# gersteinlab/REPIC-copy

Hardware: AMD Instinct MI355X
Metric: micrographs/sec (get_cliques, whole node) at 1/2/4/8 MI355X; % HBM roofline (higher is better)
Workload: dtype f64; 1 GPU; C2: {'k': 3, 'n_true': 300, 'box': 180, 'width': 4096, 'height': 4096, 'keep': 0.9, 'jit': 0.08, 'fp': 0.1}; micrographs_per_gpu=10000, scaling=weak, k=3, box_size=180, boxes_per_gpu=9030947, edges_per_gpu=11401310, cliques_per_gpu=5244495, parallelism=dp1 (micrograph shards), io=HBM-resident, steps_in_flight=3, streams=3

## Files before the change

repic-copy_amd/csrc/rgc_device.h:

```cpp
#pragma once
#pragma clang fp contract(off)
#include <hip/hip_runtime.h>
#include <stdint.h>
#include <math.h>

#include "pyset.h"

namespace rgc {

constexpr int WG = 256;
constexpr int NW = WG / 64;

template <typename T>
using gptr = __attribute__((address_space(1))) T*;
#if defined(RGC_STAMPS)
template <typename T>
__device__ __forceinline__ gptr<T> gdetach(T* p) { return (gptr<T>)p; }
__device__ __forceinline__ double sdetach(double v) { return v; }
__device__ __forceinline__ int sdetach(int v) { return v; }
__device__ __forceinline__ int64_t sdetach(int64_t v) { return v; }
#else
template <typename T>
__device__ __forceinline__ gptr<T> gdetach(T* p) {
  uint64_t v = (uint64_t)p, r;
// ... 124 lines not shown
  float r;
  asm("v_min_f32 %0, %1, %2" : "=v"(r) : "v"(a), "v"(b));
  return r;
}
__device__ __forceinline__ float wave_incl_min_f32(float v) {
  const int inf = 0x7f800000;
#define RGC_DPP_MIN(ctrl, rm, bc)                                                          \
  v = vmin_f32(v, __int_as_float(__builtin_amdgcn_update_dpp(inf, __float_as_int(v), ctrl, \
                                                             rm, 0xf, bc)))
  RGC_DPP_MIN(0x111, 0xf, false);
  RGC_DPP_MIN(0x112, 0xf, false);
  RGC_DPP_MIN(0x114, 0xf, false);
  RGC_DPP_MIN(0x118, 0xf, false);
  RGC_DPP_MIN(0x142, 0xa, false);
  RGC_DPP_MIN(0x143, 0xc, false);
#undef RGC_DPP_MIN
  return v;
}

template <int BS, typename A>
__device__ __forceinline__ int block_scan_dpp32(A* a, int n, int* lds) {
  constexpr bool PAIRS = sizeof(A) == 2;
  const int per0 = (n + BS - 1) / BS;
  const int per = PAIRS ? (per0 + 1) & ~1 : per0;
  const int c0 = min((int)threadIdx.x * per, n), c1 = min(c0 + per, n);
  uint32_t* a2 = reinterpret_cast<uint32_t*>(a);
  const int ce = PAIRS ? c0 + ((c1 - c0) & ~1) : c1;
  int s = 0;
  if constexpr (PAIRS) {
    for (int c = c0; c < ce; c += 2) {
      const uint32_t v = a2[c >> 1];
      s += (int)(v & 0xFFFFu) + (int)(v >> 16);
    }
    if (ce < c1) s += a[ce];
  } else {
    for (int c = c0; c < c1; ++c) s += a[c];
  }
  const int l = threadIdx.x & 63, w = threadIdx.x >> 6;
  const int inc = wave_incl_add32(s);
  if (l == 63) lds[w] = inc;
  __syncthreads();
  int pre = inc - s, tot = 0;
#pragma unroll
  for (int i = 0; i < BS / 64; ++i) {
    const int x = lds[i];
    pre += (i < w) ? x : 0;
    tot += x;
  }
  if constexpr (PAIRS) {
    for (int c = c0; c < ce; c += 2) {
      const uint32_t v = a2[c >> 1];
      const int p1 = pre + (int)(v & 0xFFFFu);
      a2[c >> 1] = ((uint32_t)pre & 0xFFFFu) | ((uint32_t)p1 << 16);
      pre = p1 + (int)(v >> 16);
    }
    if (ce < c1) a[ce] = (A)pre;
  } else {
    for (int c = c0; c < c1; ++c) {
      const int v = a[c];
      a[c] = (A)pre;
      pre += v;
    }
  }
  if (threadIdx.x == BS - 1) a[n] = (A)tot;
  __syncthreads();
  return tot;
}

template <int BS, typename T>
__device__ __forceinline__ T block_excl_scan_dpp(T v, T* lds, T* total) {
  const int l = threadIdx.x & 63, w = threadIdx.x >> 6;
  const T inc = wave_incl_scan(v, [](T a, T b) { return a + b; });
  if (l == 63) lds[w] = inc;
  __syncthreads();
  T pre = 0, tot = 0;
#pragma unroll
  for (int i = 0; i < BS / 64; ++i) {
    const T x = lds[i];
    pre += (i < w) ? x : (T)0;
    tot += x;
  }
  *total = tot;
  return pre + inc - v;
}

template <int BS, typename A>
__device__ __forceinline__ int64_t block_scan_dpp(A* a, int n, int64_t* lds) {
  const int per = (n + BS - 1) / BS;
  const int c0 = min((int)threadIdx.x * per, n), c1 = min(c0 + per, n);
  int64_t s = 0;
  for (int c = c0; c < c1; ++c) s += a[c];
  int64_t tot;
  int64_t pre = block_excl_scan_dpp<BS>(s, lds, &tot);
  for (int c = c0; c < c1; ++c) {
    const A v = a[c];
    a[c] = (A)pre;
    pre += v;
  }
  if (threadIdx.x == BS - 1) a[n] = (A)tot;
  __syncthreads();
  return tot;
}

template <int BS = WG>
__device__ __forceinline__ int64_t block_excl_scan(int64_t v, int64_t* lds, int64_t* total) {
  const int l = threadIdx.x & 63, w = threadIdx.x >> 6;
  int64_t inc = v;
  for (int o = 1; o < 64; o <<= 1) {
    const int64_t t = __shfl_up(inc, o, 64);
    if (l >= o) inc += t;
  }
  __syncthreads();
  if (l == 63) lds[w] = inc;
  __syncthreads();
  int64_t pre = 0, tot = 0;
  for (int i = 0; i < BS / 64; ++i) {
    if (i < w) pre += lds[i];
    tot += lds[i];
  }
  *total = tot;
  return pre + inc - v;
}

template <int BS = WG>
__device__ __forceinline__ int64_t block_scan_array(uint32_t* a, int n, int64_t* lds) {
  const int per = (n + BS - 1) / BS;
  const int c0 = min((int)threadIdx.x * per, n), c1 = min(c0 + per, n);
  int64_t s = 0;
  for (int c = c0; c < c1; ++c) s += a[c];
  int64_t tot;
  int64_t pre = block_excl_scan<BS>(s, lds, &tot);
  for (int c = c0; c < c1; ++c) {
    const uint32_t v = a[c];
    a[c] = (uint32_t)pre;
    pre += v;
  }
  __syncthreads();
  return tot;
}

template <int BS = WG>
__device__ __forceinline__ int64_t block_scan_u16(uint16_t* a, int n, int64_t* lds) {
  const int per = (n + BS - 1) / BS;
  const int c0 = min((int)threadIdx.x * per, n), c1 = min(c0 + per, n);
  int64_t s = 0;
  for (int c = c0; c < c1; ++c) s += a[c];
  int64_t tot;
  int64_t pre = block_excl_scan<BS>(s, lds, &tot);
  for (int c = c0; c < c1; ++c) {
    const uint16_t v = a[c];
    a[c] = (uint16_t)pre;
    pre += v;
  }
  __syncthreads();
  return tot;
}

__host__ __device__ __forceinline__ double overlap(double x, double y, double a, double b, double B) {
  const double xo = fmax((fmin(x, a) + B) - fmax(x, a), 0.0);
  const double yo = fmax((fmin(y, b) + B) - fmax(y, b), 0.0);
  return xo * yo;
}

__host__ __device__ __forceinline__ double jaccard(double x, double y, double a, double b, double B,
                                          double two_b2) {
  const double xo = fmax((fmin(x, a) + B) - fmax(x, a), 0.0);
// ... 241 lines not shown
```

repic-copy_amd/csrc/rgc_fused.hip:

```cpp
#pragma clang fp contract(off)

#include <type_traits>

#ifdef RGC_STAMPS
#include <hip/hip_runtime.h>
namespace rgc {
__shared__ unsigned long long g_bwait[16];
__device__ __forceinline__ void raw_barrier() {
  __builtin_amdgcn_fence(__ATOMIC_RELEASE, "workgroup");
  __builtin_amdgcn_s_barrier();
  __builtin_amdgcn_fence(__ATOMIC_ACQUIRE, "workgroup");
}
__device__ __forceinline__ void timed_barrier() {
  const unsigned long long t0 = __builtin_amdgcn_s_memtime();
  raw_barrier();
  if ((threadIdx.x & 63) == 0) g_bwait[threadIdx.x >> 6] += __builtin_amdgcn_s_memtime() - t0;
}
}
#define __syncthreads() ::rgc::timed_barrier()
#endif

#include "rgc_device.h"
#include "rgc_kernels.h"

namespace rgc {

constexpr int MAXW = 16;
constexpr int fused_rb(int nt) { return nt <= 256 ? 4 : nt >= 1024 ? 5 : 2; }
enum : unsigned { TWO_P1 = 1, TWO_P2C = 2, TWO_P3A = 4, TWO_P3B = 8, TWO_P5 = 16, TWO_P6A = 32 };
#ifndef RGC_TWO_MASK
#define RGC_TWO_MASK 0u
#endif
constexpr unsigned fused_two(int k, bool wide, int nt) {
  unsigned m = RGC_TWO_MASK;
  if (fused_rb(nt) != 2) m &= ~TWO_P1;
  if (k >= 4) m &= ~TWO_P5;
  return m;
}

struct FusedHdr {
  union {
    struct {
      double redd[MAXW];
      int64_t red64[MAXW];
      uint64_t redu[MAXW];
      int redi[MAXW];
    };
    double red4[4][MAXW];
  };
  double minx, miny, cell, inv_cell, inv_celly;
  double xbs;
  float inv_gy;
  int gx, gy, ncell, nkey;
  int E, nodes, cc_cnt, cc_max, target, V, status;
  uint32_t ccur;
  int tief[2];
  int qslot;
  int64_t C, base;
};

__host__ __device__ inline int fused_cells(int nmax) { return nmax <= 2048 ? 4 * nmax : 2 * nmax; }

__host__ __device__ inline int fwd_blocks(int nmax) { return (nmax + 63) / 64; }

__host__ __device__ inline FusedLayout fused_layout(int nmax, int ecap, bool wide) {
  FusedLayout L;
  auto al = [](int v) { return (v + 15) & ~15; };
  int o = al((int)sizeof(FusedHdr));
  L.off_sxy = o; o += al((wide ? 16 : 8) * nmax);
  L.off_cnt = o; o += al(4 * (nmax + 4));
  L.off_fwd = o; o += al(2 * (fwd_blocks(nmax) * 65 + 4));
  L.off_pos = o; o += al(2 * nmax);
  L.off_vrank = o; o += al(2 * nmax);
  L.off_dst = o; o += al(2 * ecap);
  L.off_union = o;
  L.off_cstart = o; o += al(2 * (fused_cells(nmax) + 8));
  L.off_parent = o; o += al(2 * (nmax + 8));
  L.off_scell = o; o += al(2 * nmax);
  L.off_citems = o; o += al(2 * nmax);
  L.off_flags = o; o += al(nmax);
  L.off_smark = o;
  L.total = o;
  L.off_cbuf = L.off_cstart;
  return L;
}

int fused_lds_bytes(int nmax, int ecap, bool wide) { return fused_layout(nmax, ecap, wide).total; }

struct FShared {
  void* sxy;
  uint16_t* cstart;
  uint32_t* cnt;
  uint16_t* fwd;
  uint16_t* bend;
  uint16_t* parent;
  uint16_t* citems;
  uint16_t* pos;
  uint16_t* scell;
  uint16_t* vrank;
  uint8_t* flags;
  uint16_t* dst;
  uint16_t* split;
  uint16_t* cbuf;
  double* vscore;
  bool vstaged;
  __device__ __forceinline__ int eb(int i) const { return fwd[i]; }
  __device__ __forceinline__ int ee(int i) const {
    return (i & 63) == 63 ? bend[i >> 6] : fwd[i + 1];
  }
};

template <bool W>
__device__ __forceinline__ double2 ld_xy(const FShared& S, int t) {
  if constexpr (W) {
    return reinterpret_cast<const double2*>(S.sxy)[t];
  } else {
    const float2 f = reinterpret_cast<const float2*>(S.sxy)[t];
    return make_double2((double)f.x, (double)f.y);
  }
}
template <bool W>
// ... 416 lines not shown
        for (int i = 0; i < K; ++i) e[4 + i] = c.b0 + li[i];
      }
      if (tie) return;
    } else {
      const uint32_t ord = node_order_ins<K>(ins);
      if (tie) arg = epi_tie_arg<K>(top, ord);
      if (multi) {
#pragma unroll
        for (int i = 0; i < K; ++i) c.order[j * K + i] = (uint8_t)((ord >> (4 * i)) & 15);
      }
    }
  }
  int cons = li[0];
#pragma unroll
  for (int i = 1; i < K; ++i) cons = (arg == i) ? li[i] : cons;
  c.consensus[j] = c.b0 + cons;
}

template <int K, int D, bool FILL>
struct FLevel {
  __device__ __forceinline__ static void run(FCtx<K>& c, int (&mem)[K]) {
    const int prev = mem[D - 1];
    const int lo = c.S.eb(prev);
    int hi;
    if (FILL) hi = lb16(c.S.dst, lo, c.S.ee(prev), c.pp[D + 1]);
    else hi = c.S.split[prev];
    for (int e = lo; e < hi; ++e) {
      const int h = c.S.dst[e];
      bool ok = true;
#pragma unroll
      for (int q = 0; q < D - 1; ++q) {
        if (!contains16(c.S.dst, c.S.eb(mem[q]), c.S.ee(mem[q]), h)) { ok = false; break; }
      }
      if (!ok) continue;
      mem[D] = h;
      FLevel<K, D + 1, FILL>::run(c, mem);
    }
  }
};
template <int K, bool FILL>
struct FLevel<K, K, FILL> {
  __device__ __forceinline__ static void run(FCtx<K>& c, int (&mem)[K]) {
    if (FILL) {
      const int64_t j = c.out++;
      if (j >= c.c0 && j < c.c1) {
        uint16_t* dstb = c.S.cbuf + (j - c.c0) * K;
#pragma unroll
        for (int i = 0; i < K; ++i) dstb[i] = (uint16_t)mem[i];
        c.cq_ord[j - c.c0] = 0;
      }
    } else {
      const uint32_t o = (uint32_t)c.count++;
      const uint32_t slot = atomicAdd(c.ccur, 1u);
      if (slot < (uint32_t)c.cq_cap) {
#pragma unroll
        for (int i = 0; i < K; ++i) c.S.cbuf[slot * K + i] = (uint16_t)mem[i];
        c.cq_ord[slot] = (uint16_t)o;
      }
#pragma unroll
      for (int i = 0; i < K; ++i) {
        c.S.flags[mem[i]] = 3;
      }
    }
  }
};

template <int K>
struct BfsOut {
  int64_t C;
  int lvl[K + 1];
  float fit;
};
__device__ __forceinline__ float bfs_fit(int64_t need, int64_t have) {
  return need > 0 ? (float)max(have, (int64_t)0) / (float)need : 1.0f;
}

template <bool WE>
constexpr int bfs_es() { return WE ? 8 : 4; }
__device__ __forceinline__ uint2 we_pack(const int (&mm)[4], int d, int h) {
  int t[4] = {mm[0], mm[1], mm[2], mm[3]};
  t[d] = h;
  return make_uint2((uint32_t)t[0] | ((uint32_t)t[1] << 16), (uint32_t)t[2] | ((uint32_t)t[3] << 16));
}
template <int K, int D, int NT, bool WE = false>
struct BfsLevel {
  __device__ __forceinline__ static void unpack(const uint2 v, int (&mm)[K]) {
    const int t[4] = {(int)(v.x & 0xFFFF), (int)(v.x >> 16), (int)(v.y & 0xFFFF), (int)(v.y >> 16)};
#pragma unroll
    for (int d = 0; d < D && d < 4; ++d) mm[d] = t[d];
  }
  __device__ __forceinline__ static void prefix(const char* q, const int (&lvl)[K + 1],
                                                uint32_t e, int (&mm)[K]) {
    if constexpr (WE) {
      unpack(reinterpret_cast<const uint2*>(q + lvl[D])[e], mm);
      return;
    }
    uint32_t ent = reinterpret_cast<const uint32_t*>(q + lvl[D])[e];
    mm[D - 1] = (int)(ent & 0xFFFF);
    uint32_t cur = ent >> 16;
#pragma unroll
    for (int d = D - 1; d >= 2; --d) {
      ent = reinterpret_cast<const uint32_t*>(q + lvl[d])[cur];
      mm[d - 1] = (int)(ent & 0xFFFF);
      cur = ent >> 16;
    }
    mm[0] = (int)cur;
  }

  template <bool REWALK>
  __device__ __forceinline__ static int seg_end(const FShared& S, const int (&pp)[K + 1], int m) {
    if (REWALK) return lb16(S.dst, S.eb(m), S.ee(m), pp[D + 1]);
    return S.split[m];
  }

  template <bool REWALK, typename EP>
  __device__ __forceinline__ static BfsOut<K> run(const FShared& S, FusedHdr& H, char* q,
                                                  int qbytes, BfsOut<K>& out, int64_t nD, int tid,
                                                  const int (&pp)[K + 1], const EP& ep) {
    int (&lvl)[K + 1] = out.lvl;
    constexpr int ES = bfs_es<WE>();
    const int tb = (qbytes - 8 * (int)(nD + 1)) & ~7;
    if (K >= 4) {
      const float f = fminf(bfs_fit(nD, 65535), bfs_fit((8 + ES) * nD, qbytes - lvl[D] - 8));
      out.fit = fminf(out.fit, f);
    }
    if (nD > 65535 || tb < lvl[D] + ES * (int)nD) {
      out.C = -1;
      out.fit = fminf(out.fit, 0.999f);
      return out;
    }
    uint32_t* MK = reinterpret_cast<uint32_t*>(q + tb);
    uint32_t* CN = MK + nD;
    for (int e = tid; e < nD; e += NT) {
      int mm[K];
      prefix(q, lvl, (uint32_t)e, mm);
      const int m = mm[D - 1];
      const int lo = S.eb(m), hi = seg_end<REWALK>(S, pp, m);
      uint32_t mask = 0, cnt = 0;
      typename EP::CT mc[K > 2 ? K - 2 : 1];
#pragma unroll
      for (int d = 0; d < D - 1; ++d) mc[d] = ep.pt(S, mm[d]);
      for (int t = lo; t < hi; ++t) {
        const int h = S.dst[t];
        const typename EP::CT ch = ep.pt(S, h);
        bool ok = true;
#pragma unroll
        for (int d = 0; d < D - 1; ++d) ok &= ep.edge(mc[d], ch);
        cnt += ok ? 1u : 0u;
        mask |= (ok && t - lo < 32) ? (1u << (t - lo)) : 0u;
      }
      MK[e] = mask;
      CN[e] = cnt;
    }
    __syncthreads();
    const int64_t nN = ufl(block_scan_dpp32<NT>(CN, (int)nD, H.redi));
    constexpr bool last = D + 1 == K;
    const int nb = ufl((lvl[D] + ES * (int)nD + 7) & ~7);
    if (K >= 4) {
      const float f = fminf(bfs_fit(nN, 65535), bfs_fit(nN * (last ? ES + 2 : ES), tb - nb));
      out.fit = fminf(out.fit, f);
    }
    if (nN > 65535 || nN * (last ? ES + 2 : ES) > tb - nb) {
      out.C = -1;
      out.fit = fminf(out.fit, 0.999f);
      return out;
    }
    for (int e = tid; e < nD; e += NT) {
      int mm[K];
      prefix(q, lvl, (uint32_t)e, mm);
      const int m = mm[D - 1];
      const int lo = S.eb(m), hi = seg_end<REWALK>(S, pp, m);
      const uint32_t mask = MK[e];
      uint32_t o = CN[e];
      for (int t = lo; t < hi; ++t) {
        const int h = S.dst[t];
        bool ok;
        if (t - lo < 32) {
          ok = (mask >> (t - lo)) & 1u;
        } else {
          const typename EP::CT ch = ep.pt(S, h);
          ok = true;
#pragma unroll
          for (int d = 0; d < D - 1; ++d) ok &= ep.edge(ep.pt(S, mm[d]), ch);
        }
        if (!ok) continue;
        if constexpr (WE) {
          int m4[4] = {0, 0, 0, 0};
#pragma unroll
          for (int d = 0; d < D && d < 4; ++d) m4[d] = mm[d];
          reinterpret_cast<uint2*>(q + nb)[o] = we_pack(m4, D < 4 ? D : 3, h);
        } else {
          reinterpret_cast<uint32_t*>(q + nb)[o] = ((uint32_t)e << 16) | (uint32_t)h;
        }
        if (last) {
          if (!REWALK) {
#pragma unroll
            for (int d = 0; d < K - 1; ++d) S.flags[mm[d]] = 3;
            S.flags[h] = 3;
          }
          reinterpret_cast<uint16_t*>(q + nb + ES * (int)nN)[o] = 0;
        }
        ++o;
      }
    }
    __syncthreads();
    lvl[D + 1] = nb;
    if constexpr (D + 1 < K) {
      return BfsLevel<K, D + 1, NT, WE>::template run<REWALK>(S, H, q, qbytes, out, nN, tid, pp, ep);
    } else {
      out.C = nN;
      return out;
    }
  }
};

template <int K, bool REWALK, int NT, bool WE = false, typename EP>
__device__ __forceinline__ BfsOut<K> bfs_cliques(const FShared& S, FusedHdr& H, char* q,
                                                 int qbytes, int r0, int r1, bool get_cc,
                                                 uint32_t target, int tid,
                                                 const int (&pp)[K + 1], const EP& ep) {
  BfsOut<K> out;
  out.C = -1;
  out.fit = 4.0f;
#pragma unroll
  for (int d = 0; d <= K; ++d) out.lvl[d] = 0;
  const int nr = r1 - r0;
  auto root_ok = [&](int r) {
    if (REWALK) return S.flags[r] == 3;
    return S.eb(r) < S.ee(r) && (!get_cc || S.parent[r] == target);
  };
  auto seg_end = [&](int r) {
    if (REWALK) return lb16(S.dst, S.eb(r), S.ee(r), pp[2]);
    return (int)S.split[r];
  };
  uint32_t* cnt = S.cnt;
  for (int i = tid; i < nr; i += NT) {
    const int r = r0 + i;
    cnt[i] = root_ok(r) ? (uint32_t)(seg_end(r) - S.eb(r)) : 0u;
  }
  __syncthreads();
  const int64_t n2 = ufl(block_scan_dpp32<NT>(cnt, nr, H.redi));
  constexpr bool last = K == 2;
  constexpr int ES = bfs_es<WE>();
  if (K >= 4) out.fit = fminf(bfs_fit(n2, 65535), bfs_fit(n2 * (last ? ES + 2 : ES), qbytes));
  if (n2 > 65535 || n2 * (last ? ES + 2 : ES) > qbytes) {
    out.fit = fminf(out.fit, 0.999f);
    return out;
  }
  for (int i = tid; i < nr; i += NT) {
    const int r = r0 + i;
    if (!root_ok(r)) continue;
    uint32_t o = cnt[i];
    const int se = seg_end(r);
    for (int t = S.eb(r); t < se; ++t, ++o) {
      const int h = S.dst[t];
      if constexpr (WE) reinterpret_cast<uint2*>(q)[o] = make_uint2((uint32_t)r | ((uint32_t)h << 16), 0u);
      else reinterpret_cast<uint32_t*>(q)[o] = ((uint32_t)r << 16) | (uint32_t)h;
      if (last) {
        if (!REWALK) {
          S.flags[r] = 3;
          S.flags[h] = 3;
        }
        reinterpret_cast<uint16_t*>(q + ES * (int)n2)[o] = 0;
      }
    }
  }
  __syncthreads();
  out.lvl[2] = 0;
  if constexpr (K > 2) {
    return BfsLevel<K, 2, NT, WE>::template run<REWALK>(S, H, q, qbytes, out, n2, tid, pp, ep);
  } else {
    out.C = n2;
    return out;
  }
}

constexpr int FILL_FAST = 2;

struct Stencil {
  int p, cx, y0, y1;
  double2 a;
};

template <int K, bool W>
__device__ __forceinline__ void stencil_setup(Stencil& st, int ts, const FShared& S,
                                              const GridU& H) {
  const int key = S.scell[ts];
  st.a = ld_xy<W>(S, ts);
  st.p = K;
  st.cx = 0;
  st.y0 = 0;
  st.y1 = -1;
  const int gy = H.gy, nc = H.ncell;
  if (key >= (K - 1) * nc) return;
  int p = 0;
#pragma unroll
  for (int q = 1; q < K; ++q) p += (key >= q * nc) ? 1 : 0;
  const int cell = key - p * nc;
  int cx = (int)((float)cell * H.inv_gy);
  cx += ((cx + 1) * gy <= cell) ? 1 : 0;
  cx -= (cx * gy > cell) ? 1 : 0;
  const int cy = cell - cx * gy;
  const float u = (W ? (float)(st.a.x - H.minx) : (float)st.a.x - (float)H.minx) * H.inv_cellf;
  st.p = p;
  st.cx = cx - ((u - (float)cx) < 0.5f ? 1 : 0);
  st.y0 = max(cy - 1, 0);
  st.y1 = min(cy + 1, gy - 1);
}

struct Span {
  int n0, n, o0, d;
  __device__ __forceinline__ int at(int j) const { return j + o0 + (j >= n0 ? d : 0); }
};

__device__ __forceinline__ void stencil_bounds(const Stencil& st, const FShared& S,
                                               const GridU& H, int q, int (&b)[4]) {
  const int cb = q * H.ncell + st.cx * H.gy;
  const bool ok0 = st.cx >= 0, ok1 = st.cx + 1 < H.gx;
  b[0] = S.cstart[ok0 ? cb + st.y0 : 0];
  b[1] = S.cstart[ok0 ? cb + st.y1 + 1 : 0];
  b[2] = S.cstart[ok1 ? cb + H.gy + st.y0 : 0];
  b[3] = S.cstart[ok1 ? cb + H.gy + st.y1 + 1 : 0];
}
__device__ __forceinline__ Span span_of(const int (&b)[4]) {
  Span g;
  g.n0 = b[1] - b[0];
  g.n = g.n0 + (b[3] - b[2]);
  g.o0 = b[0];
  g.d = b[2] - g.n0 - b[0];
  return g;
}

__device__ __forceinline__ void stencil_spans3(const Stencil& st, const FShared& S,
                                               const GridU& H, Span& g0, Span& g1) {
  int b0[4] = {0, 0, 0, 0}, b1[4] = {0, 0, 0, 0};
  if (st.p + 1 < 3) stencil_bounds(st, S, H, st.p + 1, b0);
  if (st.p + 2 < 3) stencil_bounds(st, S, H, st.p + 2, b1);
  g0 = span_of(b0);
  g1 = span_of(b1);
}

template <int K, typename F>
__device__ __forceinline__ void stencil_walk(const Stencil& st, const FShared& S,
                                             const GridU& H, Span& g0, Span& g1, F&& body) {
  int kk = 0;
  if constexpr (K == 3) {
    stencil_spans3(st, S, H, g0, g1);
// ... 568 lines not shown
        for (int u = 0; u < UB; ++u) {
          const int e = e0 + u * FWG;
          sv[u] = e < E ? esrc_g[e] : 0u;
        }
#pragma unroll
        for (int u = 0; u < UB; ++u) {
          const int e = e0 + u * FWG;
          if (e >= E) break;
          const uint32_t h = S.dst[e];
          S.flags[h] = 1;
          uf_union32(S.cnt, sv[u], h);
        }
      }
      __syncthreads();
    } else if (src_ok) {
      in_flight<NF_P3A, FWG>(tid, E, [&](auto it, int first) {
        constexpr int N = decltype(it)::n;
        uint32_t a[N], h[N], pa[N], ph[N];
        it.each(first, E, [&](int j, int e) { a[j] = esrc[e]; h[j] = S.dst[e]; });
        it.each(first, E, [&](int j, int) {
          pa[j] = lds_ld(S.cnt + a[j]);
          ph[j] = lds_ld(S.cnt + h[j]);
        });
        it.each(first, E, [&](int j, int) {
          S.flags[h[j]] = 1;
          uf_union32p(S.cnt, a[j], pa[j], h[j], ph[j]);
        });
      });
      __syncthreads();
    }
    cc32 = src_ok;
    if (A.eu) {
      if (tid == 0) H.base = (int64_t)atomicAdd(A.cursor + 2, (unsigned long long)E);
      __syncthreads();
      const int64_t eb = H.base;
      if (eb + E <= A.ecap_out) {
        for (int i = tid; i < n; i += FWG) {
          const double2 a = ld_xy<W>(S, i);
          for (int e = S.eb(i), e1 = S.ee(i); e < e1; ++e) {
            const int h = S.dst[e];
            const double2 b = ld_xy<W>(S, h);
            A.eu[eb + e] = b0 + S.citems[i];
            A.ev[eb + e] = b0 + S.citems[h];
            A.eji[eb + e] = jaccard(a.x, a.y, b.x, b.y, B, two_b2);
          }
        }
      }
      __syncthreads();
      if (tid == 0) H.base = 0;
    }
  }
  if (st2 != 0) {
    if (tid == 0) put_stats(A, m, st2, E, 0, 0, 0, 0, 0, 0);
    return;
  }

  STOP_AFTER(2);
  
  STAMP(6);
  in_flight<NF_P3B, FWG>(tid, n, [&](auto it, int first) {
    constexpr int N = decltype(it)::n;
    int f[N] = {}, lo[N] = {}, hi[N] = {}, v[N] = {};
    uint32_t p[N];
    it.each(first, n, [&](int j, int i) {
      f[j] = S.flags[i];
      lo[j] = S.eb(i);
      hi[j] = S.ee(i);
      if (cc32) p[j] = lds_ld(S.cnt + i);
      v[j] = next_picker_end<K>(c.pp, i);
    });
#pragma unroll
    for (int j = 0; j < N; ++j) hi[j] = f[j] ? hi[j] : lo[j];
    lb16n<N>(S.dst, lo, hi, v);
    it.each(first, n, [&](int j, int i) {
      if (!f[j]) return;
      S.split[i] = (uint16_t)lo[j];
      const uint32_t r = cc32 ? uf_find32p(S.cnt, i, p[j]) : uf_find_lds(S.parent, i);
      p16_st(S.parent + i, r);
      atomicAdd(&ccsz[r >> 1], 1u << (16 * (r & 1)));
    });
  });
  __syncthreads();
  auto cc_size = [&](uint32_t r) { return (int)((ccsz[r >> 1] >> (16 * (r & 1))) & 0xFFFF); };
  int nodes, cc_max;
  {
    int nr = 0;
    int mx = 0;
    in_flight<NF_P3B, FWG>(tid, n, [&](auto it, int first) {
      constexpr int N = decltype(it)::n;
      int f[N], p[N];
      uint32_t sz[N];
      it.each(first, n, [&](int j, int i) {
        f[j] = S.flags[i];
        p[j] = S.parent[i];
        sz[j] = ccsz[i >> 1];
      });
      it.each(first, n, [&](int j, int i) {
        if (!f[j]) return;
        nr += 1 << 16;
        if (p[j] == i) { nr += 1; mx = max(mx, (int)((sz[j] >> (16 * (i & 1))) & 0xFFFF)); }
      });
    });
    nr = wave_incl_add32(nr);
    mx = wave_incl_max32(mx);
    if ((tid & 63) == 63) { H.redi[tid >> 6] = nr; reinterpret_cast<int*>(H.redu)[tid >> 6] = mx; }
    __syncthreads();
    int t = 0;
    int m2 = 0;
#pragma unroll
    for (int w = 0; w < FNW; ++w) {
      t += H.redi[w];
      m2 = max(m2, reinterpret_cast<const int*>(H.redu)[w]);
    }
    nodes = t >> 16;
    cc_max = m2;
    if (tid == 0) { H.nodes = nodes; H.cc_cnt = t & 0xFFFF; H.cc_max = cc_max; }
  }
  const bool get_cc = (A.flags & 1) != 0;
  int target = -1;
  if (get_cc) {
    uint64_t best = ~0ULL;
    for (int i = tid; i < n; i += FWG) {
      const int e0 = S.eb(i), e1 = S.ee(i);
      if (e0 == e1) continue;
      const uint32_t r = S.parent[i];
      if (cc_size(r) != cc_max) continue;
      const int pi = picker_of<K>(c.pp, i);
      const int h0 = S.dst[e0];
      const int ph = picker_of<K>(c.pp, h0);
      const int se = lb16(S.dst, e0, e1, picker_end<K>(c.pp, h0));
      int hmin = 1 << 30;
      for (int e = e0; e < se; ++e) hmin = min(hmin, (int)S.citems[S.dst[e]]);
      const uint64_t key = ((uint64_t)pair_index(pi, ph, K) << 48) |
                           ((uint64_t)(S.citems[i] - picker_begin<K>(c.pb, pi)) << 32) |
                           ((uint64_t)(hmin - picker_begin<K>(c.pb, ph)) << 16) | r;
      best = key < best ? key : best;
    }
    best = wave_incl_scan(best, [](uint64_t a, uint64_t b) { return a < b ? a : b; });
    if ((tid & 63) == 63) H.redu[tid >> 6] = best;
    __syncthreads();
#pragma unroll
    for (int w = 0; w < FNW; ++w) best = H.redu[w] < best ? H.redu[w] : best;
    target = (int)(best & 0xFFFF);
    if (tid == 0) H.target = target;
  }

  STOP_AFTER(3);
  STAMP(7);
  c.set_order = 2 * K < nodes;
  const int n0 = c.pp[1];
  const int qoff = (L.off_dst + 2 * H.E + 15) & ~15;
  const int qbytes_lds = L.off_parent - qoff;
  char* q = smem + qoff;
  int qbytes = qbytes_lds;
  if constexpr (QG) {
    if (qslot < 0) {
      if (tid == 0) H.qslot = A.qg_base ? qg_claim(A) : -1;
      __syncthreads();
      qslot = ufl(H.qslot);
    }
    if (qslot >= 0) {
      q = A.qg_base + (size_t)qslot * (size_t)A.qg_bytes;
      qbytes = A.qg_bytes;
    }
  }
  const bool we = QG && K <= 4 && qslot >= 0;
  uint32_t* const chtab = S.cnt + n0 + 1;
  const int maxch = K >= 4 ? min(64, (n + 3 - n0) / 2 - 1) : 1;
  BfsOut<K> bo;
  int nch = 0;
  int64_t C = 0;
  {
    int r0 = 0, len = n0;
    bool ok = maxch >= 1;
    if (tid == 0) { chtab[0] = 0; chtab[1] = 0; }
    while (ok && r0 < n0) {
      len = min(len, n0 - r0);
      if (QG && K <= 4 && qslot >= 0)
        bo = bfs_cliques<K, false, NT, QG && K <= 4>(S, H, q, qbytes, r0, r0 + len, get_cc,
                                                     (uint32_t)target, tid, c.pp, ep);
      else
        bo = bfs_cliques<K, false, NT>(S, H, q, qbytes, r0, r0 + len, get_cc, (uint32_t)target,
                                       tid, c.pp, ep);
      if (bo.C < 0) {
        ok = K >= 4 && len > 1;
        len = max(1, min(len - 1, (int)((float)len * bo.fit * 0.95f)));
        continue;
      }
      if (nch == maxch) { ok = false; break; }
      C += bo.C;
      r0 += len;
      ++nch;
      if (tid == 0) { chtab[2 * nch] = (uint32_t)r0; chtab[2 * nch + 1] = (uint32_t)C; }
      len = max(len + 1, (int)((float)len * fminf(bo.fit, 2.0f) * 0.95f));
    }
    if (!ok) { nch = 0; C = 0; bo.C = -1; }
  }
  const bool bfs_ok = nch > 0;
  if (bfs_ok) {
    c.cq_cap = (int)max(bo.C, (int64_t)1);
    c.cq_ord = reinterpret_cast<uint16_t*>(q + bo.lvl[K] + (we ? 8 : 4) * (int)bo.C);
  } else {
    S.cbuf = reinterpret_cast<uint16_t*>(smem + qoff);
    c.cq_cap = 0;
    c.ccur = &H.ccur;
    for (int r = tid; r < n0; r += FWG) {
      uint32_t cntr = 0;
      if (S.eb(r) < S.ee(r) && (!get_cc || S.parent[r] == (uint32_t)target)) {
        int mem[K];
        mem[0] = r;
        c.count = 0;
        FLevel<K, 1, false>::run(c, mem);
        cntr = (uint32_t)c.count;
      }
      S.cnt[r] = cntr;
    }
    __syncthreads();
    C = block_scan_dpp<FWG>(S.cnt, n0, H.red64);
    if (tid == 0) S.cnt[n0] = (uint32_t)C;
    c.cq_cap = qbytes_lds / (2 * K + 2);
    c.cq_ord = S.cbuf + (size_t)c.cq_cap * K;
  }
  c.S.cbuf = S.cbuf;
  STAMP(8);
#ifdef RGC_STAMPS
  if (tid == 0) {
    A.stamps[(int64_t)blockIdx.x * STAMP_SLOTS + 14] = (unsigned long long)nch;
    A.stamps[(int64_t)blockIdx.x * STAMP_SLOTS + 15] = (unsigned long long)C;
  }
#endif
  unsigned long long resv = 0;
  if (tid == 0) {
    H.C = C;
    if (C == 0) {
      H.status = RGC_ST_NO_CLIQUES;
    } else if (C > 0x7fffffff) {
      H.status = RGC_ST_DEFER;
    } else {
      int vz;
      asm volatile("v_mov_b32 %0, 0" : "=v"(vz));
      resv = atomicAdd(A.cursor + vz, (unsigned long long)C);
    }
  }
  __syncthreads();

  STOP_AFTER(4);
  STAMP(9);
  if (H.status == 0) {
    uint16_t* bcnt = S.parent;
    uint32_t* bw = reinterpret_cast<uint32_t*>(S.parent);
    uint16_t* blist = S.scell;
    using CT = typename std::conditional<W, double, float>::type;
    using CT2 = typename std::conditional<W, double2, float2>::type;
    auto ld = [&](int t) -> CT2 { return reinterpret_cast<const CT2*>(S.sxy)[t]; };
    const CT minx = (CT)H.minx, xbs = (CT)H.xbs, nlast = (CT)(n - 1);
    auto xbucket = [&](CT xv) { return (int)fmin((xv - minx) * xbs, nlast); };
    for (int q = tid; q <= (n + 1) / 2; q += FWG) bw[q] = 0;
    __syncthreads();
    in_flight<NF_P5, FWG>(tid, n, [&](auto it, int first) {
      constexpr int N = decltype(it)::n;
      int f[N], q[N];
      uint32_t r[N];
      CT x[N];
      it.each(first, n, [&](int j, int t) { f[j] = S.flags[t]; x[j] = ld(t).x; });
      it.each(first, n, [&](int j, int) {
        if (f[j] != 3) return;
        q[j] = xbucket(x[j]);
        r[j] = atomicAdd(&bw[q[j] >> 1], 1u << (16 * (q[j] & 1)));
      });
      it.each(first, n, [&](int j, int t) {
        if (f[j] == 3) S.vrank[t] = (uint16_t)((r[j] >> (16 * (q[j] & 1))) & 0xFFFFu);
      });
    });
    __syncthreads();
    const int V = block_scan_dpp32<FWG>(bcnt, n, H.redi);
    if (tid == 0) { H.V = (int)V; bcnt[n] = (uint16_t)V; }
    in_flight<NF_P5, FWG>(tid, n, [&](auto it, int first) {
      constexpr int N = decltype(it)::n;
      int f[N], vr[N], bb[N];
      CT x[N];
      it.each(first, n, [&](int j, int t) {
        f[j] = S.flags[t];
        x[j] = ld(t).x;
        vr[j] = S.vrank[t];
      });
      it.each(first, n, [&](int j, int) { if (f[j] == 3) bb[j] = bcnt[xbucket(x[j])]; });
      it.each(first, n, [&](int j, int t) {
        if (f[j] == 3) blist[bb[j] + vr[j]] = (uint16_t)t;
      });
    });
    __syncthreads();
    in_flight<NF_P5, FWG>(tid, V, [&](auto it, int first) {
      constexpr int N = decltype(it)::n;
      int t[N] = {}, vi[N] = {}, lo[N] = {}, len[N] = {};
      CT2 v[N] = {};
      uint32_t rk[N];
      it.each(first, V, [&](int j, int u0) { t[j] = blist[u0]; });
      it.each(first, V, [&](int j, int) { vi[j] = S.citems[t[j]]; v[j] = ld(t[j]); });
      it.each(first, V, [&](int j, int) {
        const int b = xbucket(v[j].x);
        lo[j] = bcnt[b];
        len[j] = (int)bcnt[b + 1] - lo[j];
      });
      int ml = 0;
#pragma unroll
      for (int j = 0; j < N; ++j) { ml = max(ml, len[j]); rk[j] = lo[j]; }
#pragma nounroll
      for (int u = 0; u < ml; ++u) {
        int tu[N], ui[N];
        CT2 w[N];
#pragma unroll
        for (int j = 0; j < N; ++j) tu[j] = blist[lo[j] + (u < len[j] ? u : 0)];
#pragma unroll
        for (int j = 0; j < N; ++j) { w[j] = ld(tu[j]); ui[j] = S.citems[tu[j]]; }
#pragma unroll
        for (int j = 0; j < N; ++j)
          rk[j] += u < len[j] && ((w[j].x < v[j].x) ||
                                  (w[j].x == v[j].x &&
                                   (w[j].y < v[j].y || (w[j].y == v[j].y && ui[j] < vi[j]))));
      }
      it.each(first, V, [&](int j, int) { S.vrank[t[j]] = (uint16_t)rk[j]; });
    });
    if (tid == 0) H.base = (int64_t)resv;
    __syncthreads();
    const bool overflow = H.base + H.C > A.cap;
    if (overflow && tid == 0) H.status = RGC_ST_OVERFLOW;

    STOP_AFTER(5);
    STAMP(10);
    if (!overflow) {
    c.S.vstaged = 8 * H.V <= L.off_citems - L.off_parent;
    if (c.S.vstaged) {
      in_flight<NF_P6A, FWG>(tid, n, [&](auto it, int first) {
        constexpr int N = decltype(it)::n;
        int f[N], vr[N], li[N];
        double sc[N];
        it.each(first, n, [&](int j, int t) {
          f[j] = S.flags[t];
          vr[j] = S.vrank[t];
          li[j] = S.citems[t];
        });
// ... 292 lines not shown
```

Measured before the change: 28.60 million micrographs/s.

## Remove workgroup barriers via single-pass BFS level scans and deferred stats

When a BFS level's frontier or root count fits within one workgroup, each thread keeps its count and mask in registers and takes its offset from a register-level block scan, replacing the LDS count array plus barrier plus separate scan. The zeroing of the phase-5 bucket counters is folded into an existing barrier, and the connected-component stats reduction is moved after clique counting when components are not requested, which removes further barriers. The one-pass path also reuses cached endpoint coordinates instead of reloading them. The cost is more register pressure and extra code paths controlled by compile-time masks, and correctness relies on the reduction slots and parent buffer not being in use at the new points.

Measured after the change: 29.35 million micrographs/s (median of 6 runs). 1.03x the previous value.

```diff
diff --git a/repic-copy_amd/csrc/rgc_device.h b/repic-copy_amd/csrc/rgc_device.h
--- a/repic-copy_amd/csrc/rgc_device.h
+++ b/repic-copy_amd/csrc/rgc_device.h
@@ -230,6 +230,23 @@
   }
   *total = tot;
   return pre + inc - v;
+}
+
+template <int BS>
+__device__ __forceinline__ int block_excl_scan_add32(int v, int* lds, int* total) {
+  const int l = threadIdx.x & 63, w = threadIdx.x >> 6;
+  const int inc = wave_incl_add32(v);
+  if (l == 63) lds[w] = inc;
+  __syncthreads();
+  int pre = inc - v, tot = 0;
+#pragma unroll
+  for (int i = 0; i < BS / 64; ++i) {
+    const int x = lds[i];
+    pre += (i < w) ? x : 0;
+    tot += x;
+  }
+  *total = tot;
+  return pre;
 }
 
 template <int BS, typename A>
diff --git a/repic-copy_amd/csrc/rgc_fused.hip b/repic-copy_amd/csrc/rgc_fused.hip
--- a/repic-copy_amd/csrc/rgc_fused.hip
+++ b/repic-copy_amd/csrc/rgc_fused.hip
@@ -37,6 +37,12 @@
   if (k >= 4) m &= ~TWO_P5;
   return m;
 }
+
+enum : unsigned { BAR_P5_ZERO = 1, BAR_P3B_STATS = 2 };
+#ifndef RGC_BAR_MASK
+#define RGC_BAR_MASK 3u
+#endif
+constexpr unsigned fused_bars() { return RGC_BAR_MASK; }
 
 struct FusedHdr {
   union {
@@ -619,6 +625,15 @@
   t[d] = h;
   return make_uint2((uint32_t)t[0] | ((uint32_t)t[1] << 16), (uint32_t)t[2] | ((uint32_t)t[3] << 16));
 }
+#ifndef RGC_BFS_ONE
+#define RGC_BFS_ONE 3
+#endif
+enum : int { ONE_LEVELS = 1, ONE_ROOTS = 2, ONE_EVERY = 4 };
+constexpr bool bfs_one_trip(int k, int nt, int part) {
+  return (RGC_BFS_ONE & part) != 0 && ((RGC_BFS_ONE & ONE_EVERY) != 0 || (k <= 3 && nt <= 768));
+}
+__device__ __forceinline__ int* bfs_scan_slots(FusedHdr& H) { return reinterpret_cast<int*>(H.red64); }
+
 template <int K, int D, int NT, bool WE = false>
 struct BfsLevel {
   __device__ __forceinline__ static void unpack(const uint2 v, int (&mm)[K]) {
@@ -666,49 +681,69 @@
       out.fit = fminf(out.fit, 0.999f);
       return out;
     }
-    uint32_t* MK = reinterpret_cast<uint32_t*>(q + tb);
-    uint32_t* CN = MK + nD;
-    for (int e = tid; e < nD; e += NT) {
-      int mm[K];
-      prefix(q, lvl, (uint32_t)e, mm);
-      const int m = mm[D - 1];
-      const int lo = S.eb(m), hi = seg_end<REWALK>(S, pp, m);
-      uint32_t mask = 0, cnt = 0;
-      typename EP::CT mc[K > 2 ? K - 2 : 1];
-#pragma unroll
-      for (int d = 0; d < D - 1; ++d) mc[d] = ep.pt(S, mm[d]);
-      for (int t = lo; t < hi; ++t) {
-        const int h = S.dst[t];
-        const typename EP::CT ch = ep.pt(S, h);
-        bool ok = true;
-#pragma unroll
-        for (int d = 0; d < D - 1; ++d) ok &= ep.edge(mc[d], ch);
-        cnt += ok ? 1u : 0u;
-        mask |= (ok && t - lo < 32) ? (1u << (t - lo)) : 0u;
-      }
-      MK[e] = mask;
-      CN[e] = cnt;
-    }
-    __syncthreads();
-    const int64_t nN = ufl(block_scan_dpp32<NT>(CN, (int)nD, H.redi));
     constexpr bool last = D + 1 == K;
     const int nb = ufl((lvl[D] + ES * (int)nD + 7) & ~7);
-    if (K >= 4) {
-      const float f = fminf(bfs_fit(nN, 65535), bfs_fit(nN * (last ? ES + 2 : ES), tb - nb));
-      out.fit = fminf(out.fit, f);
-    }
-    if (nN > 65535 || nN * (last ? ES + 2 : ES) > tb - nb) {
-      out.C = -1;
-      out.fit = fminf(out.fit, 0.999f);
-      return out;
-    }
-    for (int e = tid; e < nD; e += NT) {
-      int mm[K];
-      prefix(q, lvl, (uint32_t)e, mm);
-      const int m = mm[D - 1];
-      const int lo = S.eb(m), hi = seg_end<REWALK>(S, pp, m);
-      const uint32_t mask = MK[e];
-      uint32_t o = CN[e];
+    auto next_fits = [&](int64_t nN) {
+      if (K >= 4) {
+        const float f = fminf(bfs_fit(nN, 65535), bfs_fit(nN * (last ? ES + 2 : ES), tb - nb));
+        out.fit = fminf(out.fit, f);
+      }
+      if (nN > 65535 || nN * (last ? ES + 2 : ES) > tb - nb) {
+        out.C = -1;
+        out.fit = fminf(out.fit, 0.999f);
+        return false;
+      }
+      return true;
+    };
+    auto put = [&](uint32_t e, const int (&mm)[K], int h, uint32_t o, int64_t nN) {
+      if constexpr (WE) {
+        int m4[4] = {0, 0, 0, 0};
+#pragma unroll
+        for (int d = 0; d < D && d < 4; ++d) m4[d] = mm[d];
+        reinterpret_cast<uint2*>(q + nb)[o] = we_pack(m4, D < 4 ? D : 3, h);
+      } else {
+        reinterpret_cast<uint32_t*>(q + nb)[o] = (e << 16) | (uint32_t)h;
+      }
+      if (last) {
+        if (!REWALK) {
+#pragma unroll
+          for (int d = 0; d < K - 1; ++d) S.flags[mm[d]] = 3;
+          S.flags[h] = 3;
+        }
+        reinterpret_cast<uint16_t*>(q + nb + ES * (int)nN)[o] = 0;
+      }
+    };
+    int64_t nN;
+    if (bfs_one_trip(K, NT, ONE_LEVELS) && nD <= NT) {
+      const bool act = tid < (int)nD;
+      int mm[K] = {};
+      int lo = 0, hi = 0;
+      uint32_t mask = 0, cnt = 0;
+      typename EP::CT mc[K > 2 ? K - 2 : 1] = {};
+      if (act) {
+        prefix(q, lvl, (uint32_t)tid, mm);
+        const int m = mm[D - 1];
+        lo = S.eb(m);
+        hi = seg_end<REWALK>(S, pp, m);
+#pragma unroll
+        for (int d = 0; d < D - 1; ++d) mc[d] = ep.pt(S, mm[d]);
+        for (int t = lo; t < hi; ++t) {
+          const int h = S.dst[t];
+          const typename EP::CT ch = ep.pt(S, h);
+          bool ok = true;
+#pragma unroll
+          for (int d = 0; d < D - 1; ++d) ok &= ep.edge(mc[d], ch);
+          cnt += ok ? 1u : 0u;
+          mask |= (ok && t - lo < 32) ? (1u << (t - lo)) : 0u;
+        }
+      }
+      int tot;
+      uint32_t o = (uint32_t)block_excl_scan_add32<NT>((int)cnt, bfs_scan_slots(H), &tot);
+      nN = ufl(tot);
+      if (!next_fits(nN)) {
+        __syncthreads();
+        return out;
+      }
       for (int t = lo; t < hi; ++t) {
         const int h = S.dst[t];
         bool ok;
@@ -718,26 +753,61 @@
           const typename EP::CT ch = ep.pt(S, h);
           ok = true;
 #pragma unroll
-          for (int d = 0; d < D - 1; ++d) ok &= ep.edge(ep.pt(S, mm[d]), ch);
+          for (int d = 0; d < D - 1; ++d) ok &= ep.edge(mc[d], ch);
         }
         if (!ok) continue;
-        if constexpr (WE) {
-          int m4[4] = {0, 0, 0, 0};
-#pragma unroll
-          for (int d = 0; d < D && d < 4; ++d) m4[d] = mm[d];
-          reinterpret_cast<uint2*>(q + nb)[o] = we_pack(m4, D < 4 ? D : 3, h);
-        } else {
-          reinterpret_cast<uint32_t*>(q + nb)[o] = ((uint32_t)e << 16) | (uint32_t)h;
+        put((uint32_t)tid, mm, h, o, nN);
+        ++o;
+      }
+    } else {
+      uint32_t* MK = reinterpret_cast<uint32_t*>(q + tb);
+      uint32_t* CN = MK + nD;
+      for (int e = tid; e < nD; e += NT) {
+        int mm[K];
+        prefix(q, lvl, (uint32_t)e, mm);
+        const int m = mm[D - 1];
+        const int lo = S.eb(m), hi = seg_end<REWALK>(S, pp, m);
+        uint32_t mask = 0, cnt = 0;
+        typename EP::CT mc[K > 2 ? K - 2 : 1];
+  #pragma unroll
+        for (int d = 0; d < D - 1; ++d) mc[d] = ep.pt(S, mm[d]);
+        for (int t = lo; t < hi; ++t) {
+          const int h = S.dst[t];
+          const typename EP::CT ch = ep.pt(S, h);
+          bool ok = true;
+  #pragma unroll
+          for (int d = 0; d < D - 1; ++d) ok &= ep.edge(mc[d], ch);
+          cnt += ok ? 1u : 0u;
+          mask |= (ok && t - lo < 32) ? (1u << (t - lo)) : 0u;
         }
-        if (last) {
-          if (!REWALK) {
-#pragma unroll
-            for (int d = 0; d < K - 1; ++d) S.flags[mm[d]] = 3;
-            S.flags[h] = 3;
+        MK[e] = mask;
+        CN[e] = cnt;
+      }
+      __syncthreads();
+      nN = ufl(block_scan_dpp32<NT>(CN, (int)nD, H.redi));
+      if (!next_fits(nN)) return out;
+      for (int e = tid; e < nD; e += NT) {
+        int mm[K];
+        prefix(q, lvl, (uint32_t)e, mm);
+        const int m = mm[D - 1];
+        const int lo = S.eb(m), hi = seg_end<REWALK>(S, pp, m);
+        const uint32_t mask = MK[e];
+        uint32_t o = CN[e];
+        for (int t = lo; t < hi; ++t) {
+          const int h = S.dst[t];
+          bool ok;
+          if (t - lo < 32) {
+            ok = (mask >> (t - lo)) & 1u;
+          } else {
+            const typename EP::CT ch = ep.pt(S, h);
+            ok = true;
+  #pragma unroll
+            for (int d = 0; d < D - 1; ++d) ok &= ep.edge(ep.pt(S, mm[d]), ch);
           }
-          reinterpret_cast<uint16_t*>(q + nb + ES * (int)nN)[o] = 0;
+          if (!ok) continue;
+          put((uint32_t)e, mm, h, o, nN);
+          ++o;
         }
-        ++o;
       }
     }
     __syncthreads();
@@ -771,25 +841,18 @@
     return (int)S.split[r];
   };
   uint32_t* cnt = S.cnt;
-  for (int i = tid; i < nr; i += NT) {
-    const int r = r0 + i;
-    cnt[i] = root_ok(r) ? (uint32_t)(seg_end(r) - S.eb(r)) : 0u;
-  }
-  __syncthreads();
-  const int64_t n2 = ufl(block_scan_dpp32<NT>(cnt, nr, H.redi));
   constexpr bool last = K == 2;
   constexpr int ES = bfs_es<WE>();
-  if (K >= 4) out.fit = fminf(bfs_fit(n2, 65535), bfs_fit(n2 * (last ? ES + 2 : ES), qbytes));
-  if (n2 > 65535 || n2 * (last ? ES + 2 : ES) > qbytes) {
-    out.fit = fminf(out.fit, 0.999f);
-    return out;
-  }
-  for (int i = tid; i < nr; i += NT) {
-    const int r = r0 + i;
-    if (!root_ok(r)) continue;
-    uint32_t o = cnt[i];
-    const int se = seg_end(r);
-    for (int t = S.eb(r); t < se; ++t, ++o) {
+  auto level2_fits = [&](int64_t n2) {
+    if (K >= 4) out.fit = fminf(bfs_fit(n2, 65535), bfs_fit(n2 * (last ? ES + 2 : ES), qbytes));
+    if (n2 > 65535 || n2 * (last ? ES + 2 : ES) > qbytes) {
+      out.fit = fminf(out.fit, 0.999f);
+      return false;
+    }
+    return true;
+  };
+  auto put = [&](int r, int lo, int hi, uint32_t o, int64_t n2) {
+    for (int t = lo; t < hi; ++t, ++o) {
       const int h = S.dst[t];
       if constexpr (WE) reinterpret_cast<uint2*>(q)[o] = make_uint2((uint32_t)r | ((uint32_t)h << 16), 0u);
       else reinterpret_cast<uint32_t*>(q)[o] = ((uint32_t)r << 16) | (uint32_t)h;
@@ -800,6 +863,36 @@
         }
         reinterpret_cast<uint16_t*>(q + ES * (int)n2)[o] = 0;
       }
+    }
+  };
+  int64_t n2;
+  if (bfs_one_trip(K, NT, ONE_ROOTS) && nr <= NT) {
+    const int r = r0 + tid;
+    int lo = 0, hi = 0;
+    if (tid < nr && root_ok(r)) {
+      lo = S.eb(r);
+      hi = seg_end(r);
+    }
+    int tot;
+    const uint32_t o = (uint32_t)block_excl_scan_add32<NT>(hi - lo, bfs_scan_slots(H), &tot);
+    n2 = ufl(tot);
+    if (!level2_fits(n2)) {
+      __syncthreads();
+      return out;
+    }
+    put(r, lo, hi, o, n2);
+  } else {
+    for (int i = tid; i < nr; i += NT) {
+      const int r = r0 + i;
+      cnt[i] = root_ok(r) ? (uint32_t)(seg_end(r) - S.eb(r)) : 0u;
+    }
+    __syncthreads();
+    n2 = ufl(block_scan_dpp32<NT>(cnt, nr, H.redi));
+    if (!level2_fits(n2)) return out;
+    for (int i = tid; i < nr; i += NT) {
+      const int r = r0 + i;
+      if (!root_ok(r)) continue;
+      put(r, S.eb(r), seg_end(r), cnt[i], n2);
     }
   }
   __syncthreads();
@@ -1534,7 +1627,9 @@
   });
   __syncthreads();
   auto cc_size = [&](uint32_t r) { return (int)((ccsz[r >> 1] >> (16 * (r & 1))) & 0xFFFF); };
-  int nodes, cc_max;
+  const bool get_cc = (A.flags & 1) != 0;
+  int nodes = 0, cc_max = 0;
+  int* const sred = reinterpret_cast<int*>(H.redd);
   {
     int nr = 0;
     int mx = 0;
@@ -1555,20 +1650,25 @@
     });
     nr = wave_incl_add32(nr);
     mx = wave_incl_max32(mx);
-    if ((tid & 63) == 63) { H.redi[tid >> 6] = nr; reinterpret_cast<int*>(H.redu)[tid >> 6] = mx; }
-    __syncthreads();
+    if ((tid & 63) == 63) { sred[tid >> 6] = nr; sred[MAXW + (tid >> 6)] = mx; }
+  }
+  auto cc_stats = [&]() {
     int t = 0;
     int m2 = 0;
 #pragma unroll
     for (int w = 0; w < FNW; ++w) {
-      t += H.redi[w];
-      m2 = max(m2, reinterpret_cast<const int*>(H.redu)[w]);
+      t += sred[w];
+      m2 = max(m2, sred[MAXW + w]);
     }
     nodes = t >> 16;
     cc_max = m2;
     if (tid == 0) { H.nodes = nodes; H.cc_cnt = t & 0xFFFF; H.cc_max = cc_max; }
-  }
-  const bool get_cc = (A.flags & 1) != 0;
+  };
+  const bool stats_late = (fused_bars() & BAR_P3B_STATS) != 0 && !get_cc;
+  if (!stats_late) {
+    __syncthreads();
+    cc_stats();
+  }
   int target = -1;
   if (get_cc) {
     uint64_t best = ~0ULL;
@@ -1599,7 +1699,6 @@
 
   STOP_AFTER(3);
   STAMP(7);
-  c.set_order = 2 * K < nodes;
   const int n0 = c.pp[1];
   const int qoff = (L.off_dst + 2 * H.E + 15) & ~15;
   const int qbytes_lds = L.off_parent - qoff;
@@ -1674,6 +1773,8 @@
     c.cq_ord = S.cbuf + (size_t)c.cq_cap * K;
   }
   c.S.cbuf = S.cbuf;
+  if (stats_late) cc_stats();
+  c.set_order = 2 * K < nodes;
   STAMP(8);
 #ifdef RGC_STAMPS
   if (tid == 0) {
@@ -1694,6 +1795,8 @@
       resv = atomicAdd(A.cursor + vz, (unsigned long long)C);
     }
   }
+  if (fused_bars() & BAR_P5_ZERO)
+    for (int q = tid; q <= (n + 1) / 2; q += FWG) reinterpret_cast<uint32_t*>(S.parent)[q] = 0;
   __syncthreads();
 
   STOP_AFTER(4);
@@ -1707,8 +1810,10 @@
     auto ld = [&](int t) -> CT2 { return reinterpret_cast<const CT2*>(S.sxy)[t]; };
     const CT minx = (CT)H.minx, xbs = (CT)H.xbs, nlast = (CT)(n - 1);
     auto xbucket = [&](CT xv) { return (int)fmin((xv - minx) * xbs, nlast); };
-    for (int q = tid; q <= (n + 1) / 2; q += FWG) bw[q] = 0;
-    __syncthreads();
+    if (!(fused_bars() & BAR_P5_ZERO)) {
+      for (int q = tid; q <= (n + 1) / 2; q += FWG) bw[q] = 0;
+      __syncthreads();
+    }
     in_flight<NF_P5, FWG>(tid, n, [&](auto it, int first) {
       constexpr int N = decltype(it)::n;
       int f[N], q[N];
```
